# espiriki/Garbage_Classification_RCA

Measured on AMD Instinct MI355X. Metric: train samples/sec (image+text pairs), MM-RCA ViT-B16+DistilBERT, higher is better.
Workload: dtype bf16

## Files before the change

garbage_classification_rca_amd/csrc/gemm256.hip:

```cpp
#include "common.h"
#include "lds_asm.h"
#include <type_traits>
#include <mutex>

typedef __attribute__((ext_vector_type(4))) float f32x4;
typedef __attribute__((address_space(3))) void lds_void;
typedef const __attribute__((address_space(1))) void gbl_void;

#define HT_BYTES (128 * 64 * 2)
#define STAGE_BYTES (4 * HT_BYTES)
#define LDS256_BYTES (128 * (256 * 4 + 16))
#define SLOT_A0 0
#define SLOT_A1 1
#define SLOT_B0 2
#define SLOT_B1 3

__device__ __forceinline__ int krow_f2(int row) { return (row & 3) | (((row >> 3) & 1) << 2); }

__device__ __forceinline__ void stage_half(const bf16_t* src0, const bf16_t* src1, char* lds_piece0) {
  __builtin_amdgcn_global_load_lds((gbl_void*)src0, (lds_void*)(lds_piece0), 16, 0, 0);
  __builtin_amdgcn_global_load_lds((gbl_void*)src1, (lds_void*)(lds_piece0 + 1024), 16, 0, 0);
}

template <bool F4>
__device__ __forceinline__ void stage_half_t(const bf16_t* src0, const bf16_t* src1, char* lds_piece0) {
  __builtin_amdgcn_global_load_lds((gbl_void*)src0, (lds_void*)(lds_piece0), 16, 0, 0);
  __builtin_amdgcn_global_load_lds((gbl_void*)src1, (lds_void*)(lds_piece0 + (F4 ? 8192 : 1024)), 16, 0, 0);
}

template <bool KROW, bool STRIPE = false>
__device__ __forceinline__ const bf16_t* piece_src(const bf16_t* __restrict__ base, int64_t ld, int64_t row0, int64_t rows_total,
                                                   int i, int lane, int h = 0) {
  if (!KROW) {
    const int r = 8 * i + (lane >> 3);
    const int c = (lane & 7) ^ ((r >> 1) & 7);
    int64_t gr = row0 + (STRIPE ? 64 * (r >> 5) + 32 * h + (r & 31) : r);
    if (gr > rows_total - 1) gr = rows_total - 1;
    return base + gr * ld + c * 8;
  } else {
    const int kr = 4 * i + (lane >> 4);
    const int chp = lane & 15;
    const int c = ((((chp >> 1) ^ krow_f2(kr))) << 1) | (chp & 1);
    int64_t col = row0 + (STRIPE ? 64 * (c >> 2) + 32 * h + 8 * (c & 3) : c * 8);
    if (col + 8 > rows_total) col = 0;
    return base + (int64_t)kr * ld + col;
  }
}

#define VMCNT(N) asm volatile("s_waitcnt vmcnt(" #N ")" ::: "memory")
#define BARRIER() asm volatile("s_barrier" ::: "memory")

#define MODE_SLAB (-1)
template <bool A_KROW, bool B_KROW, int MODE, bool X3 = false>
__global__ void __launch_bounds__(512, 2)
gemm_mfma256_k(const bf16_t* __restrict__ A, const bf16_t* __restrict__ B, bf16_t* __restrict__ C, const bf16_t* __restrict__ bias,
               const bf16_t* __restrict__ addend, bf16_t* __restrict__ preact, int64_t M, int64_t N, int64_t K,
               int64_t lda, int64_t ldb, int64_t ldc, int tiles_m, int tiles_n, int ksteps_base, int ksteps_rem,
               float* __restrict__ slab, float* __restrict__ colsum, int splits,
               const bf16_t* __restrict__ A_lo = nullptr, const bf16_t* __restrict__ B_lo = nullptr, int nseg = 3) {
  constexpr bool SLAB = MODE == MODE_SLAB;
  extern __shared__ __attribute__((aligned(16))) char smem[];
  const int wave = __builtin_amdgcn_readfirstlane(threadIdx.x >> 6), lane = threadIdx.x & 63;
  const int wr = wave >> 2, wc = wave & 3;

  const int nwg = tiles_m * tiles_n;
  const int total = nwg * splits;
  const int per_xcd = (total + 7) >> 3;
  const int idx = ((int)blockIdx.x & 7) * per_xcd + ((int)blockIdx.x >> 3);
  if (((int)blockIdx.x >> 3) >= per_xcd || idx >= total) return;
  const int yb = idx / nwg, wgid = idx - yb * nwg;
  const int tm = wgid / tiles_n, tn = wgid - tm * tiles_n;
  const int64_t m_blk = (int64_t)tm * 256, n_blk = (int64_t)tn * 256;
  const int64_t kbeg_v = SLAB ? 64 * ((int64_t)yb * ksteps_base + (yb < ksteps_rem ? yb : ksteps_rem)) : 0;
  const int nt = SLAB ? ksteps_base + (yb < ksteps_rem ? 1 : 0) : (int)(K / 64);
  const int ksteps_seg = (int)(K / 64);
  int issue_seg = X3 ? (int)(kbeg_v / K) : 0;
  const int64_t kbeg = X3 ? kbeg_v - (int64_t)issue_seg * K : kbeg_v;
  int issue_kt = (int)(kbeg / 64);

  f32x4 acc[2][2][4][2];
#pragma unroll
  for (int a = 0; a < 2; ++a)
#pragma unroll
    for (int b = 0; b < 2; ++b)
#pragma unroll
      for (int i = 0; i < 4; ++i)
#pragma unroll
        for (int j = 0; j < 2; ++j) acc[a][b][i][j] = (f32x4){0.f, 0.f, 0.f, 0.f};

  const int64_t a_step = A_KROW ? 64 * lda : 64, b_step = B_KROW ? 64 * ldb : 64;
  const bf16_t* pa[2][2];
  const bf16_t* pb[2][2];
  auto repoint = [&](int seg, int64_t k0) {
    const bf16_t* Ab = (X3 && seg == 1) ? A_lo : A;
    const bf16_t* Bb = (X3 && seg == 2) ? B_lo : B;
#pragma unroll
    for (int h = 0; h < 2; ++h)
#pragma unroll
      for (int ii = 0; ii < 2; ++ii) {
        pa[h][ii] = piece_src<A_KROW>(Ab, lda, m_blk + 128 * h, M, wave * 2 + ii, lane) + (A_KROW ? k0 * lda : k0);
        pb[h][ii] = piece_src<B_KROW>(Bb, ldb, n_blk + 128 * h, N, wave * 2 + ii, lane) + (B_KROW ? k0 * ldb : k0);
      }
  };
  repoint(issue_seg, kbeg);
  char* const my_piece = smem + wave * 2048;
// ... 27 lines not shown
  } else {
    const int q = l16 >> 2, p = l16 & 3, row = 8 * g + q;
#pragma unroll
    for (int j = 0; j < 2; ++j) bbase[j] = lds0 + row * 256 + ((((2 * wc + j) ^ krow_f2(row))) << 5) + p * 8;
  }
#define A_FRAG(SLOT, f, ks) read_frag<A_KROW, (SLOT) * HT_BYTES + (A_KROW ? (ks) * 8192 : (f) * 2048)>(af[f][ks], abase[A_KROW ? (f) : (ks)])
#define B_FRAG(BF, SLOT, f, ks) read_frag<B_KROW, (SLOT) * HT_BYTES + (B_KROW ? (ks) * 8192 : (f) * 2048)>(BF[f][ks], bbase[B_KROW ? (f) : (ks)])

  Frag<A_KROW> af[4][2];
  Frag<B_KROW> b0f[2][2], b1f[2][2];
  [[maybe_unused]] unsigned read_stage = 0;
#define LOAD_A(SLOT)                                                                                          \
  do {                                                                                                        \
    A_FRAG(SLOT, 0, 0); A_FRAG(SLOT, 0, 1); A_FRAG(SLOT, 1, 0); A_FRAG(SLOT, 1, 1);                           \
    A_FRAG(SLOT, 2, 0); A_FRAG(SLOT, 2, 1); A_FRAG(SLOT, 3, 0); A_FRAG(SLOT, 3, 1);                           \
  } while (0)
#define LOAD_B(BF, SLOT)                                                                                      \
  do {                                                                                                        \
    B_FRAG(BF, SLOT, 0, 0); B_FRAG(BF, SLOT, 0, 1); B_FRAG(BF, SLOT, 1, 0); B_FRAG(BF, SLOT, 1, 1);           \
  } while (0)
#define LGKM0_A() lgkm0(af)
#define LGKM0_B(BF) lgkm0(BF)
#define MFMA_QUAD(AH, BH, BF)                                                                                 \
  do {                                                                                                        \
    __builtin_amdgcn_s_setprio(1);                                                                            \
    _Pragma("unroll") for (int ks = 0; ks < 2; ++ks)                                                          \
      _Pragma("unroll") for (int i = 0; i < 4; ++i)                                                           \
        _Pragma("unroll") for (int j = 0; j < 2; ++j)                                                         \
          acc[AH][BH][i][j] = __builtin_amdgcn_mfma_f32_16x16x32_bf16(frag_val(BF[j][ks]), frag_val(af[i][ks]), acc[AH][BH][i][j], 0, 0, 0); \
    __builtin_amdgcn_s_setprio(0);                                                                            \
  } while (0)
#define END_LOAD(N)    do { if (wr) VMCNT(N); BARRIER(); __builtin_amdgcn_sched_barrier(0); } while (0)
#define END_COMPUTE(N) do { __builtin_amdgcn_sched_barrier(0); if (!wr) VMCNT(N); BARRIER(); } while (0)
#define K_TILE_G(ISS, I0, I1, I2, I3, W0, W1, W2, W3)                                                         \
  do {                                                                                                        \
    if (I0) ISS(2);                                                                                           \
    LOAD_B(b0f, SLOT_B0); LOAD_A(SLOT_A0);                                                                    \
    END_LOAD(W0);                                                                                             \
    LGKM0_B(b0f); LGKM0_A();                                                                                  \
    MFMA_QUAD(0, 0, b0f);                                                                                     \
    END_COMPUTE(W0);                                                                                          \
    if (I1) ISS(3);                                                                                           \
    LOAD_B(b1f, SLOT_B1);                                                                                     \
    END_LOAD(W1);                                                                                             \
    LGKM0_B(b1f);                                                                                             \
    MFMA_QUAD(0, 1, b1f);                                                                                     \
    END_COMPUTE(W1);                                                                                          \
    if (I2) ISS(0);                                                                                           \
    LOAD_A(SLOT_A1);                                                                                          \
    END_LOAD(W2);                                                                                             \
    LGKM0_A();                                                                                                \
    MFMA_QUAD(1, 1, b1f);                                                                                     \
    END_COMPUTE(W2);                                                                                          \
    if (I3) ISS(1);                                                                                           \
    END_LOAD(W3);                                                                                             \
    MFMA_QUAD(1, 0, b0f);                                                                                     \
    END_COMPUTE(W3);                                                                                          \
    _Pragma("unroll") for (int x = 0; x < 4; ++x) abase[x] ^= STAGE_BYTES;                                    \
    bbase[0] ^= STAGE_BYTES; bbase[1] ^= STAGE_BYTES; read_stage ^= STAGE_BYTES;                              \
  } while (0)

#define A_FRAG4(SLOT, f, pl) read_frag<false, (SLOT) * HT_BYTES + (f) * 1024>(af[f][pl], abase[pl])
#define B_FRAG4(BF, SLOT, f, pl) read_frag<false, (SLOT) * HT_BYTES + (f) * 1024>(BF[f][pl], bbase[pl])
#define LOAD_A4(SLOT)                                                                                         \
  do {                                                                                                        \
    A_FRAG4(SLOT, 0, 0); A_FRAG4(SLOT, 0, 1); A_FRAG4(SLOT, 1, 0); A_FRAG4(SLOT, 1, 1);                       \
    A_FRAG4(SLOT, 2, 0); A_FRAG4(SLOT, 2, 1); A_FRAG4(SLOT, 3, 0); A_FRAG4(SLOT, 3, 1);                       \
  } while (0)
#define LOAD_B4(BF, SLOT)                                                                                     \
  do {                                                                                                        \
    B_FRAG4(BF, SLOT, 0, 0); B_FRAG4(BF, SLOT, 0, 1); B_FRAG4(BF, SLOT, 1, 0); B_FRAG4(BF, SLOT, 1, 1);       \
  } while (0)
#define MFMA_QUAD4(AH, BH, BF)                                                                                \
  do {                                                                                                        \
    __builtin_amdgcn_s_setprio(1);                                                                            \
    _Pragma("unroll") for (int pr = 0; pr < 3; ++pr)       \
      _Pragma("unroll") for (int i = 0; i < 4; ++i)                                                           \
        _Pragma("unroll") for (int j = 0; j < 2; ++j)                                                         \
          acc[AH][BH][i][j] = __builtin_amdgcn_mfma_f32_16x16x32_bf16(frag_val(BF[j][pr == 2 ? 1 : 0]), frag_val(af[i][pr == 1 ? 1 : 0]), acc[AH][BH][i][j], 0, 0, 0); \
    __builtin_amdgcn_s_setprio(0);                                                                            \
  } while (0)
#define K_TILE_G4(ISS, I0, I1, I2, I3, W0, W1, W2, W3)                                                        \
  do {                                                                                                        \
    if (I0) ISS(2);                                                                                           \
    LOAD_B4(b0f, SLOT_B0); LOAD_A4(SLOT_A0);                                                                  \
    END_LOAD(W0);                                                                                             \
    LGKM0_B(b0f); LGKM0_A();                                                                                  \
    MFMA_QUAD4(0, 0, b0f);                                                                                    \
    END_COMPUTE(W0);                                                                                          \
// ... 9 lines not shown
    LGKM0_A();                                                                                                \
    MFMA_QUAD4(1, 1, b1f);                                                                                    \
    END_COMPUTE(W2);                                                                                          \
    if (I3) ISS(1);                                                                                           \
    END_LOAD(W3);                                                                                             \
    MFMA_QUAD4(1, 0, b0f);                                                                                    \
    END_COMPUTE(W3);                                                                                          \
    _Pragma("unroll") for (int x = 0; x < 4; ++x) abase[x] ^= STAGE_BYTES;                                    \
    bbase[0] ^= STAGE_BYTES; bbase[1] ^= STAGE_BYTES; read_stage ^= STAGE_BYTES;                              \
  } while (0)

  ISSUE(0); ISSUE(1); ISSUE(2); ISSUE(3); ISSUE(0); ISSUE(1);
  VMCNT(8);
  BARRIER();
  if (wr) BARRIER();
  __builtin_amdgcn_sched_barrier(0);

  for (int t = 0; t < nt - 2; ++t) K_TILE_G(ISSUE, 1, 1, 1, 1, 8, 8, 10, 8);
  K_TILE_G(ISSUE, 1, 1, 0, 0, 8, 8, 8, 4);
  K_TILE_G(ISSUE, 0, 0, 0, 0, 2, 0, 0, 0);
  if (!wr) BARRIER();

  if constexpr (SLAB) {
    float* dst = slab + ((int64_t)yb * nwg + (int64_t)tm * tiles_n + tn) * 65536 + wave * 8192 + lane * 4;
#pragma unroll
    for (int a = 0; a < 2; ++a)
#pragma unroll
      for (int b = 0; b < 2; ++b)
#pragma unroll
        for (int i = 0; i < 4; ++i)
#pragma unroll
          for (int j = 0; j < 2; ++j)
            *reinterpret_cast<f32x4*>(dst + (((a * 2 + b) * 4 + i) * 2 + j) * 256) = acc[a][b][i][j];
    return;
  }

}

#define EP_BASE (2 * STAGE_BYTES)
#define DS_WRITE_B128(addr, val, off) asm volatile("ds_write_b128 %0, %1 offset:%2" :: "v"(addr), "v"(val), "i"(off) : "memory")

template <bool A_KROW, bool B_KROW, int ACT, bool ADD, bool X3 = false, bool PLANES = false, bool F4 = false>
__global__ void __launch_bounds__(512, 2)
gemm_p256_k(const bf16_t* __restrict__ A, const bf16_t* __restrict__ B, bf16_t* __restrict__ C, const bf16_t* __restrict__ bias,
            const bf16_t* __restrict__ addend, bf16_t* __restrict__ preact, int64_t M, int64_t N, int64_t K,
            int64_t lda, int64_t ldb, int64_t ldc, int tiles_m, int tiles_n, float* __restrict__ colsum, int skew_ticks, int dbg,
            const bf16_t* __restrict__ A_lo = nullptr, const bf16_t* __restrict__ B_lo = nullptr, bf16_t* __restrict__ C_lo = nullptr,
            int nseg = 3, int pre16 = 0, float* __restrict__ sk_slab = nullptr, unsigned* __restrict__ sk_count = nullptr, int sk_split = 0) {
  static_assert(!X3 || (!ADD && ACT != MMRCA_ACT_MUL), "the bf16x3 form has no side-operand epilogue");
  static_assert(!F4 || (X3 && !A_KROW && !B_KROW), "the fused four-plane form is the row-major bf16x3 forward product");
  constexpr int act = ACT;
  extern __shared__ __attribute__((aligned(16))) char smem[];
  const int wave = __builtin_amdgcn_readfirstlane(threadIdx.x >> 6), lane = threadIdx.x & 63;
  const int wr = wave >> 2, wc = wave & 3;
  const int ntiles = tiles_m * tiles_n, G = (int)gridDim.x;
  const int slot = ((int)blockIdx.x & 7) * (G >> 3) + ((int)blockIdx.x >> 3);
  const bool sk_on = sk_split > 1;
  const int dp_tiles = sk_on ? (ntiles / G) * G : ntiles;
  const int my_dp = dp_tiles > slot ? (dp_tiles - slot + G - 1) / G : 0;
  const int sk_left = ntiles - dp_tiles;
  const bool has_unit = sk_on && slot < sk_left * sk_split;
  const int my_tiles = my_dp + (has_unit ? 1 : 0);
  if (my_tiles <= 0) return;
  if (skew_ticks > 0) {
    const uint64_t t0 = __builtin_amdgcn_s_memrealtime();
    const uint64_t wait = (uint64_t)skew_ticks * (((unsigned)blockIdx.x >> 3) & 3);
    while (__builtin_amdgcn_s_memrealtime() - t0 < wait) __builtin_amdgcn_s_sleep(32);
  }
  const int nt = (int)(K / (F4 ? 32 : 64));
  int unit_tile = 0, unit_part = 0, unit_k0 = 0, unit_len = nt;
// ... 463 lines not shown
  if (!(N % 256 == 0 && K % 64 == 0 && K >= 128 && a_layout == MMRCA_ROWK) || has_addend || has_colsum) return false;
  return act == MMRCA_ACT_NONE || act == MMRCA_ACT_GELU_SAVE_GRAD;
}

int mmrca_gemm256_x3_streamk_split(int64_t M, int64_t N, int64_t K, int b_layout, bool has_a_lo, bool has_b_lo, void* stream) {
  if (!(b_layout != MMRCA_KROW && has_a_lo && has_b_lo && K % 32 == 0 && K >= 64)) return 0;
  return mmrca_gemm256_streamk_split(M, N, K / 32, stream, true);
}

int mmrca_gemm256_x3(const void* A_hi, const void* A_lo, const void* B_hi, const void* B_lo, void* C, void* C_lo, const void* bias,
                     void* preact, int64_t M, int64_t N, int64_t K, int64_t lda, int64_t ldb, int64_t ldc, int b_layout, int act,
                     hipStream_t st, int pre16) {
  const bool bk = b_layout == MMRCA_KROW;
  MMRCA_REQUIRE(M * lda * 2 < (1ll << 32) && (bk ? K * ldb : N * ldb) * 2 < (1ll << 32) && M * ldc * 4 < (1ll << 32),
                "gemm_x3(mfma256): operands must be smaller than 4 GiB");
  const bool gelu = act == MMRCA_ACT_GELU_SAVE_GRAD, planes = C_lo != nullptr;
  if (!bk && A_lo && B_lo && K % 32 == 0 && K >= 64) {
    with_bools([&](auto gelu_, auto planes_) {
      launch_p256<false, false, gelu_ ? MMRCA_ACT_GELU_SAVE_GRAD : MMRCA_ACT_NONE, false, true, planes_, true>(
          A_hi, B_hi, C, bias, nullptr, preact, M, N, K, lda, ldb, ldc, nullptr, st, A_lo, B_lo, C_lo, 3, pre16);
    }, gelu, planes);
    MMRCA_CHECK_LAUNCH("gemm_x3(mfma256,fused)");
    return 0;
  }
  with_bools([&](auto bk_, auto gelu_, auto planes_) {
    launch_p256<false, bk_, gelu_ ? MMRCA_ACT_GELU_SAVE_GRAD : MMRCA_ACT_NONE, false, true, planes_>(
        A_hi, B_hi, C, bias, nullptr, preact, M, N, K, lda, ldb, ldc, nullptr, st, A_lo, B_lo, C_lo, A_lo ? (B_lo ? 3 : 2) : 1, pre16);
  }, bk, gelu, planes);
  MMRCA_CHECK_LAUNCH("gemm_x3(mfma256)");
  return 0;
}

__global__ void __launch_bounds__(256)
splitk_reduce256_k(const float* __restrict__ slab, float* __restrict__ C, int64_t ldc, int ntiles, int tiles_n, int splits, int64_t M, int64_t N) {
  const int tile = blockIdx.x >> 6;
  const int idx = ((blockIdx.x & 63) << 8) + threadIdx.x;
  const float* src = slab + (int64_t)tile * 65536 + (int64_t)idx * 4;
  f32x4 s = *reinterpret_cast<const f32x4*>(src);
  for (int k = 1; k < splits; ++k) {
    const f32x4 v = *reinterpret_cast<const f32x4*>(src + (int64_t)k * ntiles * 65536);
    s += v;
  }
  const int w = idx >> 11, f = (idx >> 6) & 31, lane = idx & 63;
  const int a = f >> 4, b = (f >> 3) & 1, i = (f >> 1) & 3, j = f & 1;
  const int wr = w >> 2, wc = w & 3, l16 = lane & 15, g = lane >> 4;
  const int row = 128 * a + 64 * wr + 16 * i + l16, col = 128 * b + 32 * wc + 16 * j + 4 * g;
  const int tm = tile / tiles_n, tn = tile % tiles_n;
  if ((int64_t)tm * 256 + row >= M || (int64_t)tn * 256 + col >= N) return;
  float* dst = C + ((int64_t)tm * 256 + row) * ldc + (int64_t)tn * 256 + col;
  f32x4 c = *reinterpret_cast<f32x4*>(dst);
  c += s;
  *reinterpret_cast<f32x4*>(dst) = c;
}

extern "C" int64_t mmrca_gemm_splitk_workspace_bytes(int64_t M, int64_t N) {
  if (M <= 0 || N <= 0 || M % 8 || N % 8) return 0;
  const int64_t tiles = ((M + 255) / 256) * ((N + 255) / 256);
  if (tiles > 256) return 0;
  return (256 / tiles) * tiles * 65536 * 4;
}

static int gemm_splitk_impl(const void* A, const void* A_lo, const void* B, const void* B_lo, float* C, void* workspace,
                           int64_t workspace_bytes, int64_t M, int64_t N, int64_t K, int64_t lda, int64_t ldb, int64_t ldc,
                           int a_layout, int b_layout, void* stream) {
  const bool x3 = A_lo != nullptr;
  const int nseg = x3 ? (B_lo ? 3 : 2) : 1;
  MMRCA_REQUIRE(A && B && C && workspace, "gemm_splitk: null operand");
  const bool ragged = M % 256 != 0 || N % 256 != 0;
  MMRCA_REQUIRE(M > 0 && N > 0 && M % 8 == 0 && N % 8 == 0 && K >= 128 && K % 64 == 0 &&
                (!ragged || (a_layout == MMRCA_KROW && b_layout == MMRCA_KROW && !A_lo)),
                "gemm_splitk: needs K %% 64 == 0, K >= 128 and M, N multiples of 256 (K-major bf16 operands: of 8) (got M=%lld N=%lld K=%lld)",
                (long long)M, (long long)N, (long long)K);
  MMRCA_REQUIRE(lda % 8 == 0 && ldb % 8 == 0 && ldc % 4 == 0 && (((uintptr_t)A | (uintptr_t)B | (uintptr_t)C | (uintptr_t)workspace) & 15) == 0,
                "gemm_splitk: operands must be 16-byte aligned");
  MMRCA_REQUIRE(lda >= (a_layout == MMRCA_ROWK ? K : M) && ldb >= (b_layout == MMRCA_ROWK ? K : N) && ldc >= N, "gemm_splitk: leading dimension too small");
  const int tiles_m = (int)((M + 255) / 256), tiles_n = (int)((N + 255) / 256), tiles = tiles_m * tiles_n;
  MMRCA_REQUIRE(tiles <= 256, "gemm_splitk: more than 256 output tiles (use mmrca_gemm)");
  const int64_t ksteps = (int64_t)nseg * (K / 64);
  int64_t splits64 = 256 / tiles;
  if (splits64 > ksteps / 2) splits64 = ksteps / 2;
  const int splits = (int)splits64;
  const int ksteps_base = (int)(ksteps / splits), ksteps_rem = (int)(ksteps % splits);
  MMRCA_REQUIRE(workspace_bytes >= (int64_t)splits * tiles * 65536 * 4, "gemm_splitk: workspace too small (%lld < %lld bytes)",
                (long long)workspace_bytes, (long long)splits * tiles * 65536 * 4);
  hipStream_t st = (hipStream_t)stream;
  const bool ak = a_layout == MMRCA_KROW, bk = b_layout == MMRCA_KROW;
#define LSLAB(AK_, BK_, X3_)                                                                                                     \
  do {                                                                                                                           \
    MMRCA_MAX_LDS(LDS256_BYTES, gemm_mfma256_k<AK_, BK_, MODE_SLAB, X3_>); \
    hipLaunchKernelGGL((gemm_mfma256_k<AK_, BK_, MODE_SLAB, X3_>), dim3((tiles * splits + 7) / 8 * 8), dim3(512), LDS256_BYTES, st, (const bf16_t*)A,      \
                       (const bf16_t*)B, (bf16_t*)nullptr, (const bf16_t*)nullptr, (const bf16_t*)nullptr, (bf16_t*)nullptr, M, N, K, \
                       lda, ldb, ldc, tiles_m, tiles_n, ksteps_base, ksteps_rem, (float*)workspace, (float*)nullptr, splits,    \
                       (const bf16_t*)A_lo, (const bf16_t*)B_lo, nseg);                                                         \
  } while (0)
  if (x3) {
    if (!ak && !bk) LSLAB(false, false, true);
    else if (!ak && bk) LSLAB(false, true, true);
    else if (ak && !bk) LSLAB(true, false, true);
    else LSLAB(true, true, true);
  } else {
    if (!ak && !bk) LSLAB(false, false, false);
    else if (!ak && bk) LSLAB(false, true, false);
    else if (ak && !bk) LSLAB(true, false, false);
    else LSLAB(true, true, false);
  }
#undef LSLAB
  MMRCA_CHECK_LAUNCH("gemm_splitk(mfma256)");
  hipLaunchKernelGGL(splitk_reduce256_k, dim3(tiles * 64), dim3(256), 0, st, (const float*)workspace, C, ldc, tiles, tiles_n, splits, M, N);
  MMRCA_CHECK_LAUNCH("gemm_splitk(reduce)");
  return 0;
}

extern "C" int mmrca_gemm_splitk(const void* A, const void* B, float* C, void* workspace, int64_t workspace_bytes, int64_t M,
                                 int64_t N, int64_t K, int64_t lda, int64_t ldb, int64_t ldc, int a_layout, int b_layout,
                                 void* stream) {
  return gemm_splitk_impl(A, nullptr, B, nullptr, C, workspace, workspace_bytes, M, N, K, lda, ldb, ldc, a_layout, b_layout, stream);
}

extern "C" int mmrca_gemm_splitk_x3(const void* A_hi, const void* A_lo, const void* B_hi, const void* B_lo, float* C, void* workspace,
                                    int64_t workspace_bytes, int64_t M, int64_t N, int64_t K, int64_t lda, int64_t ldb, int64_t ldc,
                                    int a_layout, int b_layout, void* stream) {
  MMRCA_REQUIRE(A_lo || !B_lo, "gemm_x3(splitk): a B lo plane without an A lo plane is not a supported pass set");
  return gemm_splitk_impl(A_hi, A_lo, B_hi, B_lo, C, workspace, workspace_bytes, M, N, K, lda, ldb, ldc, a_layout, b_layout, stream);
}
```

garbage_classification_rca_amd/engine.py:

```python
from __future__ import annotations

import math
from typing import Dict, List, Optional, Tuple

import torch

from . import lib as L
from . import spec as S
from .conv_engine import ConvEncoder, CONV_MODELS

import os

ALIGN = 64
CONCURRENT_ENCODERS = os.environ.get("MMRCA_CONCURRENT_ENCODERS", "1") == "1"
CLS_TAIL = os.environ.get("MMRCA_CLS_TAIL", "1") == "1"
X3_WGRAD_PASSES = int(os.environ.get("MMRCA_X3_WGRAD_PASSES", "3"))
X3_DGRAD_PASSES = int(os.environ.get("MMRCA_X3_DGRAD_PASSES", "3"))
ROWPAD = 256


def _round_up(x: int, m: int) -> int:
    return (x + m - 1) // m * m


# ... 332 lines not shown
        return t

    def release_buffers(self):
        self.buffer_generation = getattr(self, "buffer_generation", 0) + 1
        self._bufs.clear()
        self._plane_valid.clear()
        self._plane_fresh.clear()
        self._saved = None
        if self.conv is not None:
            self.conv.release()

    def _lin_fwd(self, x, wkey, bkey, out, M, N, K, act=L.ACT_NONE, preact=None, addend=None, wnumel=None):
        if self.x3:
            b = self.arena.view(bkey) if wnumel is None else self.arena.p[self.arena.offsets[bkey][0]:self.arena.offsets[bkey][0] + N]
            po = isinstance(out, Planes)
            L.gemm_x3(self._split(x, M, K), self.Wx3(wkey, wnumel), out.hi if po else out, C_lo=(out.lo if po else None), bias=b, addend=addend,
                      preact=preact, M=M, N=N, K=K, lda=K, ldb=K, ldc=N, a_layout=L.ROWK, b_layout=L.ROWK, act=act, impl=self.gemm_impl)
            return
        w = self.W(wkey) if wnumel is None else self.Wflat(wkey, wnumel)
        b = self.W(bkey) if wnumel is None else self.Wflat(bkey, N)
        L.gemm(x, w, out, bias=b, addend=addend, preact=preact, M=M, N=N, K=K, lda=K, ldb=K, ldc=N,
               a_layout=L.ROWK, b_layout=L.ROWK, act=act, dtype=self.dt, impl=self.gemm_impl)

    def _lin_bwd(self, dy, x, wkey, bkey, dx, M, N, K, addend=None, wnumel=None, gelu_h=None, bias_done=False, gelu_db=None):
        Mk = _round_up(M, 64)
        gw = self.G(wkey) if wnumel is None else self.Gflat(wkey, wnumel)
        gb = self.G(bkey) if wnumel is None else self.Gflat(bkey, N)
        if self.x3 and not self.x3f:
            return self._lin_bwd_x3(dy, x, wkey, dx, M, N, K, Mk, gw, gb, addend, wnumel, gelu_h, bias_done, gelu_db)
        if self.x3f:
            x = self._hi(x, M, K)
        bdt = self.bdt
        if self.gemm_impl == L.IMPL_AUTO and L.gemm_splitk_ok(N, K, Mk, bdt):
            L.gemm_splitk(dy, x, gw, self._splitk_ws(), M=N, N=K, K=Mk, lda=N, ldb=K, ldc=K)
        else:
            L.gemm(dy, x, gw, M=N, N=K, K=Mk, lda=N, ldb=K, ldc=K, a_layout=L.KROW, b_layout=L.KROW, accum=True, dtype=bdt,
                   impl=self.gemm_impl)
        if not bias_done:
            L.colsum_accum(dy, gb, M, N, N, bdt)
        if dx is not None:
            w = self.Wb(wkey, wnumel)
            fuse = gelu_h is not None
            L.gemm(dy, w, dx, addend=addend, preact=(gelu_h if fuse else None), M=M, N=K, K=N, lda=N, ldb=K, ldc=K,
                   a_layout=L.ROWK, b_layout=L.KROW, act=(L.ACT_MUL if fuse else L.ACT_NONE), dtype=bdt,
                   impl=self.gemm_impl, colsum=(gelu_db if fuse else None))

    def _lin_bwd_x3(self, dy, x, wkey, dx, M, N, K, Mk, gw, gb, addend, wnumel, gelu_h, bias_done, gelu_db):
        dyp = self._split(dy, M, N)
        xp = self._split(x, M, K, reuse=True)
        wg_a, wg_b = (dyp, xp) if X3_WGRAD_PASSES >= 3 else ((dyp, (xp[0], None)) if X3_WGRAD_PASSES == 2 else ((dyp[0], None), (xp[0], None)))
        if self.gemm_impl == L.IMPL_AUTO and L.gemm_splitk_ok(N, K, Mk, L.BF16):
            L.gemm_splitk_x3(wg_a, wg_b, gw, self._splitk_ws(), M=N, N=K, K=Mk, lda=N, ldb=K, ldc=K)
        else:
            L.gemm_x3(wg_a, wg_b, gw, M=N, N=K, K=Mk, lda=N, ldb=K, ldc=K, a_layout=L.KROW, b_layout=L.KROW, accum=True)
        if not bias_done:
            if isinstance(dy, Planes):
                raise L.MmrcaError("bf16x3: the bias gradient of a two-plane dY must come from its producer (bias_done)")
            L.colsum_accum(dy, gb, M, N, N, self.dt)
        if dx is not None:
            fuse = gelu_h is not None
            po = isinstance(dx, Planes)
            wp = self.Wx3(wkey, wnumel)
            dg_a, dg_b = (dyp, wp) if X3_DGRAD_PASSES >= 3 else ((dyp, (wp[0], None)) if X3_DGRAD_PASSES == 2 else ((dyp[0], None), (wp[0], None)))
            L.gemm_x3(dg_a, dg_b, dx.hi if po else dx, C_lo=(dx.lo if po else None), addend=addend,
                      preact=(gelu_h if fuse else None), colsum=(gelu_db if fuse else None),
                      M=M, N=K, K=N, lda=N, ldb=K, ldc=K, a_layout=L.ROWK, b_layout=L.KROW, act=(L.ACT_MUL if fuse else L.ACT_NONE),
                      impl=self.gemm_impl)
# ... 474 lines not shown
```

garbage_classification_rca_amd/lib.py:

```python
from __future__ import annotations

import ctypes as C
import os
import subprocess
from typing import Optional

import torch

_HERE = os.path.dirname(os.path.abspath(__file__))
LIB_PATH = os.path.join(_HERE, "libmmrca.so")

F32, BF16 = 0, 1
ACT_NONE, ACT_GELU, ACT_GELU_BWD, ACT_GELU_SAVE_GRAD, ACT_MUL, ACT_GELU_SAVE_GRAD_BF16 = 0, 1, 2, 3, 4, 5
ROWK, KROW = 0, 1
IMPL_AUTO, IMPL_REF, IMPL_MFMA, IMPL_MFMA256, IMPL_MFMA_PERSIST, IMPL_MFMA_BK32, IMPL_MFMA_1STAGE, IMPL_MFMA_TALL, IMPL_MFMA_256W, IMPL_MFMA_256X4 = 0, 1, 2, 3, 4, 5, 6, 7, 8, 9

HEAD_FIELDS = [f"{blk}_{leaf}" for blk in ("sai", "sat", "c1", "c2")
               for leaf in ("wq", "bq", "wk", "bk", "wv", "bv", "g", "b")] + ["fin_w", "fin_b"]


class HeadPtrs(C.Structure):
    _fields_ = [(n, C.c_void_p) for n in HEAD_FIELDS]


class MmrcaError(RuntimeError):
    pass


def build_library(force: bool = False) -> str:
    src_dir = os.path.join(_HERE, "csrc")
    cmd = ["make", "-C", src_dir, "-j8"]
    if force:
        subprocess.run(["make", "-C", src_dir, "clean"], check=True, capture_output=True)
    r = subprocess.run(cmd, capture_output=True, text=True)
    if r.returncode != 0 or not os.path.exists(LIB_PATH):
        raise MmrcaError("building libmmrca.so failed:\n" + r.stdout[-4000:] + r.stderr[-4000:])
    return LIB_PATH


_lib = None

_i64, _i32, _f32, _vp, _u64 = C.c_int64, C.c_int, C.c_float, C.c_void_p, C.c_uint64
_SIGS = {
    "mmrca_gemm": [_vp] * 6 + [_i64] * 6 + [_i32] * 6 + [_vp],
    "mmrca_gemm_colsum": [_vp] * 7 + [_i64] * 6 + [_i32] * 5 + [_vp],
    "mmrca_gemm_rows": [_vp] * 7 + [_i64] * 8 + [_i32] * 5 + [_vp],
    "mmrca_gemm_splitk": [_vp] * 4 + [_i64] * 7 + [_i32] * 2 + [_vp],
    "mmrca_gemm_streamk_workspace": [_vp, _i64, _vp],
    "mmrca_gemm_streamk_config": [_i32, _i32, _i32],
    "mmrca_gemm_x3": [_vp] * 10 + [_i64] * 6 + [_i32] * 5 + [_vp],
    "mmrca_gemm_splitk_x3": [_vp] * 6 + [_i64] * 7 + [_i32] * 2 + [_vp],
    "mmrca_split_f32": [_vp, _vp, _vp, _i64, _vp],
    "mmrca_sgd_step_x3": [_vp, _vp, _vp, _vp, _i64, _f32, _f32, _f32, _vp],
    "mmrca_adamw_step_x3": [_vp] * 6 + [_i64] + [_f32] * 5 + [_i32, _f32, _vp],
    "mmrca_nchw_to_rows": [_vp, _vp, _i32, _i32, _i32, _i32, _i32, _vp],
    "mmrca_im2row3x3": [_vp, _vp, _i32, _i32, _i32, _i32, _i32, _i64, _i32, _vp],
    "mmrca_col2im3x3": [_vp, _vp, _i32, _i32, _i32, _i32, _i32, _i64, _i32, _vp],
    "mmrca_im2row3x3_tap": [_vp, _vp, _i32, _i32, _i32, _i32, _i32, _i64, _i32, _vp],
    "mmrca_col2im3x3_tap": [_vp, _vp, _i32, _i32, _i32, _i32, _i32, _i64, _i32, _vp],
    "mmrca_dwconv3x3_fwd": [_vp, _vp, _vp, _i32, _i32, _i32, _i32, _i32, _i32, _vp],
    "mmrca_dwconv3x3_bwd_ws": [_vp, _vp, _vp, _vp, _vp, _i32, _i32, _i32, _i32, _i32, _i32, _vp, _i64, _vp],
    "mmrca_dwconv3x3_bwd": [_vp, _vp, _vp, _vp, _vp, _i32, _i32, _i32, _i32, _i32, _i32, _vp],
    "mmrca_dwconv5x5_fwd": [_vp, _vp, _vp, _i32, _i32, _i32, _i32, _i32, _i32, _vp],
    "mmrca_dwconv5x5_bwd_ws": [_vp, _vp, _vp, _vp, _vp, _i32, _i32, _i32, _i32, _i32, _i32, _vp, _i64, _vp],
    "mmrca_conv3x3_fwd": [_vp, _vp, _vp, _vp, _vp, _vp, _i32, _i32, _i32, _i32, _i32, _i32, _vp],
    "mmrca_conv_bn_finish": [_vp, _vp, _vp, _i32, _i32, _i32, _vp, _vp, _vp, _vp, _i32, _f32, _f32, _vp],
    "mmrca_conv3x3_wgrad": [_vp, _vp, _vp, _i32, _i32, _i32, _i32, _i32, _i32, _vp],
    "mmrca_gemm_bnstats": [_vp, _vp, _vp, _i64, _i64, _i64, _i64, _i64, _i64, _i32, _vp, _vp, _vp, _vp],
    "mmrca_bn_finish_sums": [_vp, _vp, _vp, _i64, _i64, _vp, _vp, _vp, _vp, _i32, _f32, _f32, _vp],
    "mmrca_bn_act_bwd_sums": [_vp, _vp, _vp, _vp, _vp, _vp, _vp, _vp, _vp, _vp, _i64, _i32, _i32, _i32, _i32, _vp],
    "mmrca_se_dx": [_vp, _vp, _vp, _vp, _i32, _i32, _i32, _i32, _vp, _vp, _vp, _vp, _vp, _i32, _vp, _vp],
    "mmrca_bn_act_fwd_res": [_vp, _vp, _vp, _vp, _vp, _vp, _vp, _vp, _i64, _i32, _i32, _i64, _i32, _vp],
    "mmrca_bn_moments": [_vp, _vp, _vp, _vp, _i64, _i32, _i64, _i32, _vp],
    "mmrca_bn_act_fwd_fin": [_vp] * 13 + [_i64, _i32, _i32, _i64, _f32, _f32, _i32, _vp],
    "mmrca_bn_stats": [_vp, _vp, _vp, _vp, _vp, _i64, _i32, _i64, _f32, _f32, _i32, _i32, _vp],
    "mmrca_bn_stats_ws": [_vp, _vp, _vp, _vp, _vp, _i64, _i32, _i64, _f32, _f32, _i32, _i32, _vp, _i64, _i32, _vp],
    "mmrca_bn_stats_fused": [_vp, _vp, _vp, _vp, _vp, _i64, _i32, _i64, _f32, _f32, _i32, _vp, _i32, _vp],
    "mmrca_bn_act_bwd_ws": [_vp] * 10 + [_i64, _i32, _i32, _i32, _i32, _vp, _i64, _i32, _vp],
    "mmrca_bn_act_fwd": [_vp] * 6 + [_i64, _i32, _i32, _i32, _vp],
    "mmrca_bn_act_bwd": [_vp] * 10 + [_i64, _i32, _i32, _i32, _i32, _vp],
# ... 170 lines not shown
    if rows_readable is not None:
        if accum:
            raise MmrcaError("gemm: rows_readable is not available in accumulate mode")
        _check(load().mmrca_gemm_rows(ptr(A), ptr(B), ptr(Cout), ptr(bias), ptr(addend), ptr(preact), ptr(colsum), M, N, K, lda, ldb, ldc,
                                      int(rows_readable[0]), int(rows_readable[1]), a_layout, b_layout, act, dtype, impl, stream_ptr()),
               "mmrca_gemm_rows")
        return
    prof = GEMM_PROFILE is not None and (gemm_is_mfma(M, N, K, a_layout, dtype, impl) or (dtype == F32 and impl != IMPL_REF))
    timed = prof or CONV_PROFILE is not None
    if timed:
        e0, e1 = torch.cuda.Event(enable_timing=True), torch.cuda.Event(enable_timing=True)
        e0.record()
    if colsum is not None:
        if accum:
            raise MmrcaError("gemm: colsum is not available in accumulate mode")
        _check(load().mmrca_gemm_colsum(ptr(A), ptr(B), ptr(Cout), ptr(bias), ptr(addend), ptr(preact), ptr(colsum), M, N, K,
                                        lda, ldb, ldc, a_layout, b_layout, act, dtype, impl, stream_ptr()), "mmrca_gemm_colsum")
    else:
        _check(load().mmrca_gemm(ptr(A), ptr(B), ptr(Cout), ptr(bias), ptr(addend), ptr(preact), M, N, K, lda, ldb, ldc,
                                 a_layout, b_layout, act, int(accum), dtype, impl, stream_ptr()), "mmrca_gemm")
    if timed:
        e1.record()
    if prof:
        GEMM_PROFILE.append((2.0 * M * N * K, (a_layout, b_layout, int(accum)), e0, e1, (M, N, K, act)))
    if CONV_PROFILE is not None:
        es = _esz(dtype)
        side = (1 if addend is not None else 0) + (1 if preact is not None else 0)
        nbytes = int((M * K + N * K) * es + M * N * ((4 if accum else es) + side * es))
        CONV_PROFILE.append(("GEMM (1x1 conv / patch matrix / text encoder)", nbytes, e0, e1))
        if GEMM_SHAPES is not None:
            GEMM_SHAPES.append((M, N, K, a_layout, b_layout, int(accum), nbytes, e0, e1))


SPLITK_WS_BYTES = 64 << 20


def gemm_splitk_ok(M, N, K, dtype):
    return dtype == BF16 and M % 256 == 0 and N % 256 == 0 and K % 64 == 0 and K >= 128 and (M // 256) * (N // 256) <= 256


def gemm_splitk_ragged_ok(M, N, K, dtype):
    return (dtype == BF16 and M % 8 == 0 and N % 8 == 0 and K % 64 == 0 and K >= 128
            and ((M + 255) // 256) * ((N + 255) // 256) <= 256)


def gemm_splitk(A, B, Cout, workspace, *, M, N, K, lda, ldb, ldc, a_layout=KROW, b_layout=KROW):
    _dev(A, "gemm_splitk A")
    prof = GEMM_PROFILE is not None
    if prof:
        e0, e1 = torch.cuda.Event(enable_timing=True), torch.cuda.Event(enable_timing=True)
        e0.record()
    _check(load().mmrca_gemm_splitk(ptr(A), ptr(B), ptr(Cout), ptr(workspace), workspace.numel() * workspace.element_size(),
                                    M, N, K, lda, ldb, ldc, a_layout, b_layout, stream_ptr()), "mmrca_gemm_splitk")
    if prof:
        e1.record()
        GEMM_PROFILE.append((2.0 * M * N * K, (a_layout, b_layout, 1), e0, e1, (M, N, K, ACT_NONE)))
    if CONV_PROFILE is not None:
        CONV_PROFILE.append(("GEMM (1x1 conv / patch matrix / text encoder)", int((M * K + N * K) * 2 + M * N * 4), None, None))


def gemm_x3(A, B, Cout, *, C_lo=None, bias=None, addend=None, preact=None, colsum=None, M, N, K, lda, ldb, ldc, a_layout=ROWK,
            b_layout=ROWK, act=ACT_NONE, accum=False, impl=IMPL_AUTO):
    _dev(A[0], "gemm_x3 A")
    if not accum:
        streamk_workspace(M, N, A[0].device)
    prof = GEMM_PROFILE is not None
    if prof:
        e0, e1 = torch.cuda.Event(enable_timing=True), torch.cuda.Event(enable_timing=True)
        e0.record()
    _check(load().mmrca_gemm_x3(ptr(A[0]), ptr(A[1]), ptr(B[0]), ptr(B[1]), ptr(Cout), ptr(C_lo), ptr(bias), ptr(addend), ptr(preact),
                                ptr(colsum), M, N, K, lda, ldb, ldc, a_layout, b_layout, act, int(accum), impl, stream_ptr()),
           "mmrca_gemm_x3")
    if prof:
        e1.record()
        GEMM_PROFILE.append((6.0 * M * N * K, (a_layout, b_layout, int(accum)), e0, e1, (M, N, K, act)))


def gemm_splitk_x3(A, B, Cout, workspace, *, M, N, K, lda, ldb, ldc, a_layout=KROW, b_layout=KROW):
    _dev(A[0], "gemm_splitk_x3 A")
    prof = GEMM_PROFILE is not None
    if prof:
        e0, e1 = torch.cuda.Event(enable_timing=True), torch.cuda.Event(enable_timing=True)
        e0.record()
    _check(load().mmrca_gemm_splitk_x3(ptr(A[0]), ptr(A[1]), ptr(B[0]), ptr(B[1]), ptr(Cout), ptr(workspace),
                                       workspace.numel() * workspace.element_size(), M, N, K, lda, ldb, ldc, a_layout, b_layout,
                                       stream_ptr()), "mmrca_gemm_splitk_x3")
    if prof:
        e1.record()
        GEMM_PROFILE.append((6.0 * M * N * K, (a_layout, b_layout, 1), e0, e1, (M, N, K, ACT_NONE)))
# ... 503 lines not shown
```

include/mmrca.h:

```cpp
#ifndef MMRCA_H
#define MMRCA_H
#include <stdint.h>
#ifdef __cplusplus
extern "C" {
#endif

enum { MMRCA_F32 = 0, MMRCA_BF16 = 1 };
enum { MMRCA_ACT_NONE = 0, MMRCA_ACT_GELU = 1,
       MMRCA_ACT_GELU_BWD = 2,
       MMRCA_ACT_GELU_SAVE_GRAD = 3,
       MMRCA_ACT_MUL = 4,
       MMRCA_ACT_GELU_SAVE_GRAD_BF16 = 5 };
enum { MMRCA_ROWK = 0, MMRCA_KROW = 1 };
enum { MMRCA_GEMM_AUTO = 0, MMRCA_GEMM_REF = 1, MMRCA_GEMM_MFMA = 2 ,
       MMRCA_GEMM_MFMA256 = 3 ,
       MMRCA_GEMM_MFMA_PERSIST = 4 ,
       MMRCA_GEMM_MFMA_BK32 = 5 ,
       MMRCA_GEMM_MFMA_1STAGE = 6 ,
       MMRCA_GEMM_MFMA_TALL = 7 ,
       MMRCA_GEMM_MFMA_256W = 8 ,
       MMRCA_GEMM_MFMA_256X4 = 9  };

const char* mmrca_last_error(void);
int mmrca_version(void);

int mmrca_seed_epoch_set(const uint64_t* device_value, uint64_t value, void* stream);
int mmrca_sd_rowscale(const float* p, float* out, int n, int B, uint64_t seed, void* stream);
int mmrca_debug_set(int flags);
int mmrca_bn_flat_set(int mode);
int mmrca_debug_attn_stamps(void* buf);

int mmrca_gemm(const void* A, const void* B, void* C, const void* bias, const void* addend, void* preact,
               int64_t M, int64_t N, int64_t K, int64_t lda, int64_t ldb, int64_t ldc,
               int a_layout, int b_layout, int act, int out_f32_accum, int dtype, int impl, void* stream);
int mmrca_gemm_colsum(const void* A, const void* B, void* C, const void* bias, const void* addend, void* preact,
                      float* colsum, int64_t M, int64_t N, int64_t K, int64_t lda, int64_t ldb, int64_t ldc,
                      int a_layout, int b_layout, int act, int dtype, int impl, void* stream);

int64_t mmrca_gemm_bnstats_slots(int64_t M);
int mmrca_gemm_bnstats(const void* A, const void* B, void* C, int64_t M, int64_t N, int64_t K, int64_t lda, int64_t ldb, int64_t ldc,
                       int dtype, const float* shift, float* s1, float* s2, void* stream);
int mmrca_bn_finish_sums(const float* s1, const float* s2, const float* shift, int64_t nslots, int64_t rows, float* mean, float* rstd,
                         float* running_mean, float* running_var, int C, float eps, float momentum, void* stream);
int mmrca_gemm_rows(const void* A, const void* B, void* C, const void* bias, const void* addend, void* preact,
                    float* colsum, int64_t M, int64_t N, int64_t K, int64_t lda, int64_t ldb, int64_t ldc,
                    int64_t a_rows_readable, int64_t side_rows_readable, int a_layout, int b_layout, int act, int dtype,
                    int impl, void* stream);

int64_t mmrca_gemm_streamk_workspace_bytes(void);
int mmrca_gemm_streamk_workspace(void* workspace, int64_t bytes, void* stream);
int mmrca_gemm_streamk_config(int max_split, int min_ksteps, int bf16_products);

int64_t mmrca_gemm_splitk_workspace_bytes(int64_t M, int64_t N);
int mmrca_gemm_splitk(const void* A, const void* B, float* C, void* workspace, int64_t workspace_bytes, int64_t M,
                      int64_t N, int64_t K, int64_t lda, int64_t ldb, int64_t ldc, int a_layout, int b_layout, void* stream);

int mmrca_gemm_x3(const void* A_hi, const void* A_lo, const void* B_hi, const void* B_lo, void* C, void* C_lo,
                  const void* bias, const void* addend, void* preact, float* colsum, int64_t M, int64_t N, int64_t K,
                  int64_t lda, int64_t ldb, int64_t ldc, int a_layout, int b_layout, int act, int out_f32_accum,
                  int impl, void* stream);
int mmrca_gemm_splitk_x3(const void* A_hi, const void* A_lo, const void* B_hi, const void* B_lo, float* C, void* workspace,
                         int64_t workspace_bytes, int64_t M, int64_t N, int64_t K, int64_t lda, int64_t ldb, int64_t ldc,
                         int a_layout, int b_layout, void* stream);
int mmrca_split_f32(const float* src, void* hi, void* lo, int64_t n, void* stream);

int mmrca_colsum_accum(const void* dY, float* db, int64_t M, int64_t N, int64_t ld, int dtype, void* stream);

int mmrca_gelu_bwd(const void* dG, const void* H, void* dH, int64_t n, int dtype, void* stream);
int mmrca_gelu_bwd_colsum(const void* dG, const void* H, void* dH, float* db, int64_t M, int64_t N, int64_t ld,
                          int dtype, void* stream);

int mmrca_nchw_to_rows(const float* images, void* x, int B, int C, int H, int W, int dtype, void* stream);
int mmrca_im2row3x3(const void* x, void* col, int B, int H, int W, int C, int stride, int64_t ldk, int dtype, void* stream);
int mmrca_col2im3x3(const void* dcol, void* dx, int B, int H, int W, int C, int stride, int64_t ldk, int dtype, void* stream);
int mmrca_im2row3x3_tap(const void* x, void* col, int B, int H, int W, int C, int stride, int64_t ldk, int dtype, void* stream);
int mmrca_col2im3x3_tap(const void* dcol, void* dx, int B, int H, int W, int C, int stride, int64_t ldk, int dtype, void* stream);
int64_t mmrca_conv3x3_stat_slots(int B, int H, int W);
int mmrca_conv3x3_fwd(const void* x, const void* w_tap, void* z, float* part_mean, float* part_m2, float* part_cnt, int B, int H,
                      int W, int Cin, int Cout, int dtype, void* stream);
int mmrca_conv_bn_finish(float* part_mean, float* part_m2, float* part_cnt, int B, int H, int W, float* mean, float* rstd,
                         float* running_mean, float* running_var, int C, float eps, float momentum, void* stream);
int mmrca_conv3x3_wgrad(const void* dz, const void* x, float* dw_tap, int B, int H, int W, int Cin, int Cout, int dtype,
                        void* stream);
int mmrca_dwconv3x3_fwd(const void* x, const void* w, void* y, int B, int H, int W, int C, int stride, int dtype, void* stream);
int mmrca_dwconv3x3_bwd(const void* dy, const void* x, const void* w, void* dx, float* dw, int B, int H, int W, int C, int stride,
                        int dtype, void* stream);
int mmrca_dwconv3x3_bwd_ws(const void* dy, const void* x, const void* w, void* dx, float* dw, int B, int H, int W, int C, int stride,
                           int dtype, void* ws, int64_t ws_bytes, void* stream);
// ... 191 lines not shown
```

Measured before the change: 7034.

## Fuse bias-gradient column sums into split-K weight-gradient GEMM

Adds a BIAS variant of the split-K 256-tile GEMM. For tiles with tn==0 it sums the already-loaded A fragments (dY) using bf16 dot2 with ones, writes per-split partial bias sums into extra workspace, and has the reduce kernel fold those into db. The weight-gradient path calls this variant when the bias gradient is not yet computed, which removes a separate colsum pass over dY. The cost is extra dot2 work and some register pressure in the first tile column, plus a slightly larger workspace.

Result: no change. 7098, median of 6 (+0.9%).

```diff
diff --git a/garbage_classification_rca_amd/csrc/gemm256.hip b/garbage_classification_rca_amd/csrc/gemm256.hip
--- a/garbage_classification_rca_amd/csrc/gemm256.hip
+++ b/garbage_classification_rca_amd/csrc/gemm256.hip
@@ -47,11 +47,29 @@
   }
 }
 
+typedef __attribute__((ext_vector_type(2))) __bf16 bf16x2;
+__device__ __forceinline__ float dot2_ones(bf16x2 v, float s) {
+  return __builtin_amdgcn_fdot2_f32_bf16(v, (bf16x2){(__bf16)1.0f, (__bf16)1.0f}, s, false);
+}
+template <int I>
+__device__ __forceinline__ float bsum_frag(const Frag<true> (&af)[4][2], float s) {
+#pragma unroll
+  for (int ks = 0; ks < 2; ++ks) {
+    s = dot2_ones(__builtin_shufflevector(af[I][ks].lo, af[I][ks].lo, 0, 1), s);
+    s = dot2_ones(__builtin_shufflevector(af[I][ks].lo, af[I][ks].lo, 2, 3), s);
+    s = dot2_ones(__builtin_shufflevector(af[I][ks].hi, af[I][ks].hi, 0, 1), s);
+    s = dot2_ones(__builtin_shufflevector(af[I][ks].hi, af[I][ks].hi, 2, 3), s);
+  }
+  return s;
+}
+template <int I>
+__device__ __forceinline__ float bsum_frag(const Frag<false> (&)[4][2], float s) { return s; }
+
 #define VMCNT(N) asm volatile("s_waitcnt vmcnt(" #N ")" ::: "memory")
 #define BARRIER() asm volatile("s_barrier" ::: "memory")
 
 #define MODE_SLAB (-1)
-template <bool A_KROW, bool B_KROW, int MODE, bool X3 = false>
+template <bool A_KROW, bool B_KROW, int MODE, bool X3 = false, bool BIAS = false>
 __global__ void __launch_bounds__(512, 2)
 gemm_mfma256_k(const bf16_t* __restrict__ A, const bf16_t* __restrict__ B, bf16_t* __restrict__ C, const bf16_t* __restrict__ bias,
                const bf16_t* __restrict__ addend, bf16_t* __restrict__ preact, int64_t M, int64_t N, int64_t K,
@@ -71,6 +89,9 @@
   const int yb = idx / nwg, wgid = idx - yb * nwg;
   const int tm = wgid / tiles_n, tn = wgid - tm * tiles_n;
   const int64_t m_blk = (int64_t)tm * 256, n_blk = (int64_t)tn * 256;
+  static_assert(!BIAS || (SLAB && A_KROW && !X3), "bias sums: split-K form, K-major A, plain bf16");
+  [[maybe_unused]] const int bsel = (BIAS && tn == 0) ? wc : 4;
+  [[maybe_unused]] float bsum[2] = {0.f, 0.f};
   const int64_t kbeg_v = SLAB ? 64 * ((int64_t)yb * ksteps_base + (yb < ksteps_rem ? yb : ksteps_rem)) : 0;
   const int nt = SLAB ? ksteps_base + (yb < ksteps_rem ? 1 : 0) : (int)(K / 64);
   const int ksteps_seg = (int)(K / 64);
@@ -164,6 +185,18 @@
   } while (0)
 #define END_LOAD(N)    do { if (wr) VMCNT(N); BARRIER(); __builtin_amdgcn_sched_barrier(0); } while (0)
 #define END_COMPUTE(N) do { __builtin_amdgcn_sched_barrier(0); if (!wr) VMCNT(N); BARRIER(); } while (0)
+#define BSUM_HOOK(AH)                                                                                         \
+  do {                                                                                                        \
+    if constexpr (BIAS) {                                                                                     \
+      switch (bsel) {                                                                                         \
+        case 0: bsum[AH] = bsum_frag<0>(af, bsum[AH]); break;                                                 \
+        case 1: bsum[AH] = bsum_frag<1>(af, bsum[AH]); break;                                                 \
+        case 2: bsum[AH] = bsum_frag<2>(af, bsum[AH]); break;                                                 \
+        case 3: bsum[AH] = bsum_frag<3>(af, bsum[AH]); break;                                                 \
+        default: break;                                                                                       \
+      }                                                                                                       \
+    }                                                                                                         \
+  } while (0)
 #define K_TILE_G(ISS, I0, I1, I2, I3, W0, W1, W2, W3)                                                         \
   do {                                                                                                        \
     if (I0) ISS(2);                                                                                           \
@@ -177,6 +210,7 @@
     END_LOAD(W1);                                                                                             \
     LGKM0_B(b1f);                                                                                             \
     MFMA_QUAD(0, 1, b1f);                                                                                     \
+    BSUM_HOOK(0);                                                                                             \
     END_COMPUTE(W1);                                                                                          \
     if (I2) ISS(0);                                                                                           \
     LOAD_A(SLOT_A1);                                                                                          \
@@ -187,6 +221,7 @@
     if (I3) ISS(1);                                                                                           \
     END_LOAD(W3);                                                                                             \
     MFMA_QUAD(1, 0, b0f);                                                                                     \
+    BSUM_HOOK(1);                                                                                             \
     END_COMPUTE(W3);                                                                                          \
     _Pragma("unroll") for (int x = 0; x < 4; ++x) abase[x] ^= STAGE_BYTES;                                    \
     bbase[0] ^= STAGE_BYTES; bbase[1] ^= STAGE_BYTES; read_stage ^= STAGE_BYTES;                              \
@@ -262,10 +297,24 @@
 #pragma unroll
           for (int j = 0; j < 2; ++j)
             *reinterpret_cast<f32x4*>(dst + (((a * 2 + b) * 4 + i) * 2 + j) * 256) = acc[a][b][i][j];
+    if constexpr (BIAS) {
+      if (bsel < 4) {
+        float* bdst = slab + (int64_t)splits * nwg * 65536 + ((int64_t)yb * tiles_m + tm) * 256 + 64 * wr + 16 * wc + l16;
+#pragma unroll
+        for (int ah = 0; ah < 2; ++ah) {
+          float v = bsum[ah];
+          v += __shfl_xor(v, 16);
+          v += __shfl_xor(v, 32);
+          if (g == 0) bdst[128 * ah] = v;
+        }
+      }
+    }
     return;
   }
 
 }
+#undef BSUM_HOOK
+#define BSUM_HOOK(AH) do { } while (0)
 
 #define EP_BASE (2 * STAGE_BYTES)
 #define DS_WRITE_B128(addr, val, off) asm volatile("ds_write_b128 %0, %1 offset:%2" :: "v"(addr), "v"(val), "i"(off) : "memory")
@@ -795,7 +844,17 @@
 }
 
 __global__ void __launch_bounds__(256)
-splitk_reduce256_k(const float* __restrict__ slab, float* __restrict__ C, int64_t ldc, int ntiles, int tiles_n, int splits, int64_t M, int64_t N) {
+splitk_reduce256_k(const float* __restrict__ slab, float* __restrict__ C, int64_t ldc, int ntiles, int tiles_n, int splits, int64_t M,
+                   int64_t N, float* __restrict__ db, int tiles_m) {
+  if ((int)blockIdx.x >= ntiles * 64) {
+    const int64_t j = (int64_t)((int)blockIdx.x - ntiles * 64) * 256 + threadIdx.x;
+    if (!db || j >= (int64_t)tiles_m * 256 || j >= M) return;
+    const float* src = slab + (int64_t)splits * ntiles * 65536 + j;
+    float s = src[0];
+    for (int k = 1; k < splits; ++k) s += src[(int64_t)k * tiles_m * 256];
+    db[j] += s;
+    return;
+  }
   const int tile = blockIdx.x >> 6;
   const int idx = ((blockIdx.x & 63) << 8) + threadIdx.x;
   const float* src = slab + (int64_t)tile * 65536 + (int64_t)idx * 4;
@@ -825,7 +884,7 @@
 
 static int gemm_splitk_impl(const void* A, const void* A_lo, const void* B, const void* B_lo, float* C, void* workspace,
                            int64_t workspace_bytes, int64_t M, int64_t N, int64_t K, int64_t lda, int64_t ldb, int64_t ldc,
-                           int a_layout, int b_layout, void* stream) {
+                           int a_layout, int b_layout, void* stream, float* db = nullptr) {
   const bool x3 = A_lo != nullptr;
   const int nseg = x3 ? (B_lo ? 3 : 2) : 1;
   MMRCA_REQUIRE(A && B && C && workspace, "gemm_splitk: null operand");
@@ -844,14 +903,17 @@
   if (splits64 > ksteps / 2) splits64 = ksteps / 2;
   const int splits = (int)splits64;
   const int ksteps_base = (int)(ksteps / splits), ksteps_rem = (int)(ksteps % splits);
-  MMRCA_REQUIRE(workspace_bytes >= (int64_t)splits * tiles * 65536 * 4, "gemm_splitk: workspace too small (%lld < %lld bytes)",
-                (long long)workspace_bytes, (long long)splits * tiles * 65536 * 4);
+  const int64_t ws_need = (int64_t)splits * tiles * 65536 * 4 + (db ? (int64_t)splits * tiles_m * 256 * 4 : 0);
+  MMRCA_REQUIRE(workspace_bytes >= ws_need, "gemm_splitk: workspace too small (%lld < %lld bytes)", (long long)workspace_bytes,
+                (long long)ws_need);
+  MMRCA_REQUIRE(!db || (a_layout == MMRCA_KROW && b_layout == MMRCA_KROW && !x3 && ((uintptr_t)db & 3) == 0),
+                "gemm_splitk_bias: needs K-major bf16 operands (plain bf16, not bf16x3)");
   hipStream_t st = (hipStream_t)stream;
   const bool ak = a_layout == MMRCA_KROW, bk = b_layout == MMRCA_KROW;
-#define LSLAB(AK_, BK_, X3_)                                                                                                     \
+#define LSLAB(AK_, BK_, X3_, ...)                                                                                                \
   do {                                                                                                                           \
-    MMRCA_MAX_LDS(LDS256_BYTES, gemm_mfma256_k<AK_, BK_, MODE_SLAB, X3_>); \
-    hipLaunchKernelGGL((gemm_mfma256_k<AK_, BK_, MODE_SLAB, X3_>), dim3((tiles * splits + 7) / 8 * 8), dim3(512), LDS256_BYTES, st, (const bf16_t*)A,      \
+    MMRCA_MAX_LDS(LDS256_BYTES, gemm_mfma256_k<AK_, BK_, MODE_SLAB, X3_, ##__VA_ARGS__>); \
+    hipLaunchKernelGGL((gemm_mfma256_k<AK_, BK_, MODE_SLAB, X3_, ##__VA_ARGS__>), dim3((tiles * splits + 7) / 8 * 8), dim3(512), LDS256_BYTES, st, (const bf16_t*)A, \
                        (const bf16_t*)B, (bf16_t*)nullptr, (const bf16_t*)nullptr, (const bf16_t*)nullptr, (bf16_t*)nullptr, M, N, K, \
                        lda, ldb, ldc, tiles_m, tiles_n, ksteps_base, ksteps_rem, (float*)workspace, (float*)nullptr, splits,    \
                        (const bf16_t*)A_lo, (const bf16_t*)B_lo, nseg);                                                         \
@@ -861,6 +923,8 @@
     else if (!ak && bk) LSLAB(false, true, true);
     else if (ak && !bk) LSLAB(true, false, true);
     else LSLAB(true, true, true);
+  } else if (db) {
+    LSLAB(true, true, false, true);
   } else {
     if (!ak && !bk) LSLAB(false, false, false);
     else if (!ak && bk) LSLAB(false, true, false);
@@ -869,7 +933,8 @@
   }
 #undef LSLAB
   MMRCA_CHECK_LAUNCH("gemm_splitk(mfma256)");
-  hipLaunchKernelGGL(splitk_reduce256_k, dim3(tiles * 64), dim3(256), 0, st, (const float*)workspace, C, ldc, tiles, tiles_n, splits, M, N);
+  hipLaunchKernelGGL(splitk_reduce256_k, dim3(tiles * 64 + (db ? tiles_m : 0)), dim3(256), 0, st, (const float*)workspace, C, ldc, tiles,
+                     tiles_n, splits, M, N, db, tiles_m);
   MMRCA_CHECK_LAUNCH("gemm_splitk(reduce)");
   return 0;
 }
@@ -878,6 +943,13 @@
                                  int64_t N, int64_t K, int64_t lda, int64_t ldb, int64_t ldc, int a_layout, int b_layout,
                                  void* stream) {
   return gemm_splitk_impl(A, nullptr, B, nullptr, C, workspace, workspace_bytes, M, N, K, lda, ldb, ldc, a_layout, b_layout, stream);
+}
+
+extern "C" int mmrca_gemm_splitk_bias(const void* A, const void* B, float* C, float* db, void* workspace, int64_t workspace_bytes,
+                                      int64_t M, int64_t N, int64_t K, int64_t lda, int64_t ldb, int64_t ldc, int a_layout,
+                                      int b_layout, void* stream) {
+  MMRCA_REQUIRE(db, "gemm_splitk_bias: null db");
+  return gemm_splitk_impl(A, nullptr, B, nullptr, C, workspace, workspace_bytes, M, N, K, lda, ldb, ldc, a_layout, b_layout, stream, db);
 }
 
 extern "C" int mmrca_gemm_splitk_x3(const void* A_hi, const void* A_lo, const void* B_hi, const void* B_lo, float* C, void* workspace,
diff --git a/garbage_classification_rca_amd/engine.py b/garbage_classification_rca_amd/engine.py
--- a/garbage_classification_rca_amd/engine.py
+++ b/garbage_classification_rca_amd/engine.py
@@ -388,7 +388,11 @@
             x = self._hi(x, M, K)
         bdt = self.bdt
         if self.gemm_impl == L.IMPL_AUTO and L.gemm_splitk_ok(N, K, Mk, bdt):
-            L.gemm_splitk(dy, x, gw, self._splitk_ws(), M=N, N=K, K=Mk, lda=N, ldb=K, ldc=K)
+            if not bias_done and Mk == M:
+                L.gemm_splitk_bias(dy, x, gw, gb, self._splitk_ws(), M=N, N=K, K=Mk, lda=N, ldb=K, ldc=K)
+                bias_done = True
+            else:
+                L.gemm_splitk(dy, x, gw, self._splitk_ws(), M=N, N=K, K=Mk, lda=N, ldb=K, ldc=K)
         else:
             L.gemm(dy, x, gw, M=N, N=K, K=Mk, lda=N, ldb=K, ldc=K, a_layout=L.KROW, b_layout=L.KROW, accum=True, dtype=bdt,
                    impl=self.gemm_impl)
diff --git a/garbage_classification_rca_amd/lib.py b/garbage_classification_rca_amd/lib.py
--- a/garbage_classification_rca_amd/lib.py
+++ b/garbage_classification_rca_amd/lib.py
@@ -46,6 +46,7 @@
     "mmrca_gemm_colsum": [_vp] * 7 + [_i64] * 6 + [_i32] * 5 + [_vp],
     "mmrca_gemm_rows": [_vp] * 7 + [_i64] * 8 + [_i32] * 5 + [_vp],
     "mmrca_gemm_splitk": [_vp] * 4 + [_i64] * 7 + [_i32] * 2 + [_vp],
+    "mmrca_gemm_splitk_bias": [_vp] * 5 + [_i64] * 7 + [_i32] * 2 + [_vp],
     "mmrca_gemm_streamk_workspace": [_vp, _i64, _vp],
     "mmrca_gemm_streamk_config": [_i32, _i32, _i32],
     "mmrca_gemm_x3": [_vp] * 10 + [_i64] * 6 + [_i32] * 5 + [_vp],
@@ -282,7 +283,7 @@
             GEMM_SHAPES.append((M, N, K, a_layout, b_layout, int(accum), nbytes, e0, e1))
 
 
-SPLITK_WS_BYTES = 64 << 20
+SPLITK_WS_BYTES = (64 << 20) + (256 << 10)
 
 
 def gemm_splitk_ok(M, N, K, dtype):
@@ -305,6 +306,21 @@
     if prof:
         e1.record()
         GEMM_PROFILE.append((2.0 * M * N * K, (a_layout, b_layout, 1), e0, e1, (M, N, K, ACT_NONE)))
+    if CONV_PROFILE is not None:
+        CONV_PROFILE.append(("GEMM (1x1 conv / patch matrix / text encoder)", int((M * K + N * K) * 2 + M * N * 4), None, None))
+
+
+def gemm_splitk_bias(A, B, Cout, db, workspace, *, M, N, K, lda, ldb, ldc):
+    _dev(A, "gemm_splitk_bias A")
+    prof = GEMM_PROFILE is not None
+    if prof:
+        e0, e1 = torch.cuda.Event(enable_timing=True), torch.cuda.Event(enable_timing=True)
+        e0.record()
+    _check(load().mmrca_gemm_splitk_bias(ptr(A), ptr(B), ptr(Cout), ptr(db), ptr(workspace), workspace.numel() * workspace.element_size(),
+                                         M, N, K, lda, ldb, ldc, KROW, KROW, stream_ptr()), "mmrca_gemm_splitk_bias")
+    if prof:
+        e1.record()
+        GEMM_PROFILE.append((2.0 * M * N * K, (KROW, KROW, 1), e0, e1, (M, N, K, ACT_NONE)))
     if CONV_PROFILE is not None:
         CONV_PROFILE.append(("GEMM (1x1 conv / patch matrix / text encoder)", int((M * K + N * K) * 2 + M * N * 4), None, None))
 
diff --git a/include/mmrca.h b/include/mmrca.h
--- a/include/mmrca.h
+++ b/include/mmrca.h
@@ -54,6 +54,8 @@
 int64_t mmrca_gemm_splitk_workspace_bytes(int64_t M, int64_t N);
 int mmrca_gemm_splitk(const void* A, const void* B, float* C, void* workspace, int64_t workspace_bytes, int64_t M,
                       int64_t N, int64_t K, int64_t lda, int64_t ldb, int64_t ldc, int a_layout, int b_layout, void* stream);
+int mmrca_gemm_splitk_bias(const void* A, const void* B, float* C, float* db, void* workspace, int64_t workspace_bytes, int64_t M,
+                           int64_t N, int64_t K, int64_t lda, int64_t ldb, int64_t ldc, int a_layout, int b_layout, void* stream);
 
 int mmrca_gemm_x3(const void* A_hi, const void* A_lo, const void* B_hi, const void* B_lo, void* C, void* C_lo,
                   const void* bias, const void* addend, void* preact, float* colsum, int64_t M, int64_t N, int64_t K,
```
